# ctxnn/GenConViT

Hardware: AMD Instinct MI355X
Metric: frames/sec (224x224, ed+vae forward) (higher is better)
Workload: dtype f16

## Files before the change

### genconvit_amd/csrc/api.hip

```cpp
#include "../../include/genconvit_hip.h"

#include <dlfcn.h>

#include <cstdio>
#include <cstdlib>
#include <cstring>
#include <map>
#include <mutex>
#include <set>
#include <sstream>
#include <vector>

#include "fused_mlp.h"
#include "gemm.h"
#include "mlp_pair.h"
#include "xs_mlp.h"
#include "kernels.h"
#include "net.h"

namespace gcv {
static thread_local std::string g_err;
void set_error(const std::string& msg) { g_err = msg; }
const char* get_error() { return g_err.c_str(); }

// ... 144 lines not shown
  a.lnp_w = l->w; a.lnp_b = l->b; a.lnp_eps = l->eps; a.lnp_nseg = l->nseg;
  for (int i = 0; i < l->nseg && i < 4; ++i) {
    a.lnp_tok0[i] = l->tok0[i]; a.lnp_hw[i] = l->hw[i]; a.lnp_wd[i] = l->wd[i]; a.lnp_out0[i] = l->out0[i];
  }
}
template <typename T>
static int k_mlp_dispatch(int C, const void* x, const void* w1, const float* b1, const float* w2_f32, const float* b2,
                          const float* gamma, const void* resid, void* out, int M, hipStream_t s, int iters = 0,
                          float* ms = nullptr, const LnpSpec* lnp = nullptr) {
  struct DevBuf {
    void* p = nullptr;
    hipStream_t s;
    explicit DevBuf(hipStream_t st) : s(st) {}
    ~DevBuf() { if (p) { (void)hipStreamSynchronize(s); (void)hipFree(p); } }
  };
  struct Ev {
    hipEvent_t e = nullptr;
    ~Ev() { if (e) (void)hipEventDestroy(e); }
  };
  DevBuf w2c(s), w1f(s), hid(s);
  GCV_CHECK_HIP(hipMalloc(&w2c.p, (size_t)4 * C * C * 2));
  auto timed = [&](auto&& f, float* avg) -> int {
    if (iters <= 0) return f();
    Ev e0, e1;
    GCV_CHECK_HIP(hipEventCreate(&e0.e));
    GCV_CHECK_HIP(hipEventCreate(&e1.e));
    GCV_TRY(f());
    GCV_CHECK_HIP(hipEventRecord(e0.e, s));
    for (int i = 0; i < iters; ++i) GCV_TRY(f());
    GCV_CHECK_HIP(hipEventRecord(e1.e, s));
    GCV_CHECK_HIP(hipEventSynchronize(e1.e));
    float t = 0.0f;
    GCV_CHECK_HIP(hipEventElapsedTime(&t, e0.e, e1.e));
    if (avg) *avg = t / (float)iters;
    return 0;
  };
  if (ms) ms[0] = ms[1] = ms[2] = 0.0f;
  if (lnp) {
    GCV_REQUIRE(lnp->nseg >= 1 && lnp->nseg <= 4 && lnp->w && lnp->b && lnp->tok0 && lnp->hw && lnp->wd && lnp->out0,
                "fused MLP with LN-patchify epilogue: 1..4 segments and their tables");
    GCV_REQUIRE((C == 96 && fused_mlp_res_applies(C, M)) || xs_mlp_default(C),
                "the LN-patchify epilogue exists at C = 96 (M >= 65536 tokens) and C = 192");
    int64_t covered = 0;
    for (int i = 0; i < lnp->nseg; ++i) {
      const int end = i + 1 < lnp->nseg ? lnp->tok0[i + 1] : M;
      const int wd = lnp->wd[i], hw = lnp->hw[i];
      GCV_REQUIRE(wd > 0 && hw > 0 && hw % wd == 0 && wd % 2 == 0 && (hw / wd) % 2 == 0 && lnp->tok0[i] == covered &&
                      end > lnp->tok0[i] && (end - lnp->tok0[i]) % hw == 0 && lnp->out0[i] * 4 == lnp->tok0[i],
                  "LN-patchify segments: contiguous whole images with even height and width");
      covered = end;
    }
  }
  if (mlp_pair_supported(C)) {
    GCV_CHECK_HIP(hipMalloc(&w1f.p, (size_t)4 * C * C * 2));
    GCV_CHECK_HIP(hipMalloc(&hid.p, mlp_pair_hidden_bytes(M, C)));
    GCV_TRY((launch_pack_w1_frag<T, T>((const T*)w1, (T*)w1f.p, C, s)));
    GCV_TRY((launch_pack_w2_frag<T, float>(w2_f32, gamma, (T*)w2c.p, C, s)));
    MlpPairArgs a{x, w1f.p, b1, w2c.p, b2, gamma, resid, out, hid.p, M};
    if (iters > 0) {
      GCV_TRY(timed([&] { return launch_xs_pw1<T>(a, C, s); }, ms ? ms + 1 : nullptr));
      GCV_TRY(timed([&] { return launch_pw2f<T>(a, C, s); }, ms ? ms + 2 : nullptr));
    }
    return timed([&] { return launch_mlp_pair<T>(a, C, s); }, ms);
  }
  static const bool legacy = exp_env("GCV_MLP_LEGACY") != nullptr;
  if (xs_mlp_default(C) && !legacy) {
    GCV_CHECK_HIP(hipMalloc(&w1f.p, xs_mlp_packed_elems(C) * sizeof(T)));
    GCV_TRY((launch_pack_xs_mlp<T, float>((const T*)w1, w2_f32, (T*)w1f.p, C, s)));
    XsMlpArgs xa{x, w1f.p, b1, b2, gamma, resid, out, M};
    set_lnp(xa, lnp);
    return timed([&] { return launch_xs_mlp<T>(xa, C, s); }, ms);
  }
  MlpArgs a{x, w1, b1, w2c.p, b2, gamma, resid, out, M};
  set_lnp(a, lnp);
  GCV_TRY(launch_pack_w2_chunks<T>(w2_f32, (T*)w2c.p, C, s));
  return timed([&] { return launch_fused_mlp<T>(a, C, s); }, ms);
}

extern "C" {

const char* gcv_last_error(void) { return get_error(); }

struct DeviceGuard {
  int prev = -1;
  explicit DeviceGuard(int dev) {
    if (hipGetDevice(&prev) != hipSuccess) prev = -1;
    if (prev != dev) (void)hipSetDevice(dev); else prev = -1;
  }
  ~DeviceGuard() { if (prev >= 0) (void)hipSetDevice(prev); }
};

int gcv_create(gcv_handle** out, int device, int dtype, int max_batch) {
  GCV_REQUIRE(out != nullptr, "null handle pointer");
  *out = nullptr;
  GCV_REQUIRE(max_batch >= 1 && max_batch <= 512, "max_batch must be in [1,512]");
  int ndev = 0;
  GCV_CHECK_HIP(hipGetDeviceCount(&ndev));
  GCV_REQUIRE(device >= 0 && device < ndev, "no such HIP device");
  hipDeviceProp_t prop;
  GCV_CHECK_HIP(hipGetDeviceProperties(&prop, device));
  GCV_REQUIRE(std::string(prop.gcnArchName).rfind("gfx950", 0) == 0,
              std::string("kernels are built for gfx950 only, device is ") + prop.gcnArchName);
  NetBase* net = nullptr;
  switch (dtype) {
    case GCV_F32:  net = make_net_f32(); break;
    case GCV_BF16: net = make_net_bf16(); break;
    case GCV_F16:  net = make_net_f16(); break;
    default: set_error("dtype must be GCV_F32, GCV_BF16 or GCV_F16"); return -2;
  }
  net->device = device;
  net->dtype = dtype;
// ... 401 lines not shown
```

### genconvit_amd/csrc/gemm.h

```cpp
#pragma once
#include <type_traits>

#include "common.h"

namespace gcv {

enum { A_PLAIN = 0, A_IM2COL3_POOL = 1, A_IM2COL3_S2 = 2 };
enum { EPI_BIAS_ACT = 0, EPI_RESID = 1, EPI_POOL4 = 2, EPI_CONVT = 3, EPI_SPLITK = 4 };

struct GemmArgs {
  const void* A;
  const void* Wt;
  void* C;
  const float* bias;
  const float* gamma;
  const void* resid;
  float* partial;
  int M, N, K;
  int lda, ldc;
  int act;
  int splitk;
  int k_per_split;
  int H, W;
  int cin_log2;
  int cout_log2;
};

typedef float f32x4 __attribute__((ext_vector_type(4)));
typedef float f32x16 __attribute__((ext_vector_type(16)));
typedef _Float16 f16x8 __attribute__((ext_vector_type(8)));
typedef __bf16 bf16x8 __attribute__((ext_vector_type(8)));

template <typename T> struct Mfma;
template <> struct Mfma<float> {
  __device__ static __forceinline__ void run(const u32x4& a, const u32x4& b, f32x16& acc) {
    const f32x4 af = __builtin_bit_cast(f32x4, a), bf = __builtin_bit_cast(f32x4, b);
#pragma unroll
    for (int j = 0; j < 4; ++j) acc = __builtin_amdgcn_mfma_f32_32x32x2f32(af[j], bf[j], acc, 0, 0, 0);
  }
};
template <> struct Mfma<half_t> {
  __device__ static __forceinline__ void run(const u32x4& a, const u32x4& b, f32x16& acc) {
    acc = __builtin_amdgcn_mfma_f32_32x32x16_f16(__builtin_bit_cast(f16x8, a), __builtin_bit_cast(f16x8, b), acc, 0, 0, 0);
  }
};
template <> struct Mfma<bf16_t> {
  __device__ static __forceinline__ void run(const u32x4& a, const u32x4& b, f32x16& acc) {
    acc = __builtin_amdgcn_mfma_f32_32x32x16_bf16(__builtin_bit_cast(bf16x8, a), __builtin_bit_cast(bf16x8, b), acc, 0, 0, 0);
  }
};

__device__ __forceinline__ float erf_fast(float x) {
  const float a = fabsf(x);
  const float t = __builtin_amdgcn_rcpf(fmaf(0.3275911f, a, 1.0f));
  float p = fmaf(1.061405429f, t, -1.453152027f);
  p = fmaf(p, t, 1.421413741f);
  p = fmaf(p, t, -0.284496736f);
  p = fmaf(p, t, 0.254829592f);
  p *= t;
  const float e = __builtin_amdgcn_exp2f(a * a * -1.4426950408889634f);
  return copysignf(fmaf(-p, e, 1.0f), x);
// ... 518 lines not shown
```

### genconvit_amd/csrc/gemm_bf16.hip

```cpp
#include "gemm_impl.h"
namespace gcv { template int launch_gemm<bf16_t>(const GemmArgs&, int, int, hipStream_t); }
```

### genconvit_amd/csrc/gemm_f16.hip

```cpp
#include "gemm_impl.h"
namespace gcv { template int launch_gemm<half_t>(const GemmArgs&, int, int, hipStream_t); }

GCV_GLDS_STAMP_READER
```

### genconvit_amd/csrc/gemm_glds.h

```cpp
#pragma once
#include "gemm.h"

namespace gcv {

#ifndef GCV_GLDS_STAGES
#define GCV_GLDS_STAGES 2
#endif
constexpr int kGldsBM = 128, kGldsBN = 192;
template <int BKB> struct GldsRing { static constexpr int stages = BKB == 64 ? GCV_GLDS_STAGES : 2; };

template <typename T, int BKB = 64> struct GldsSmem {
  static constexpr int kStage = (kGldsBM + kGldsBN) * BKB;
  static constexpr int kMain = GldsRing<BKB>::stages * kStage;
  static constexpr int kEpiRow = kGldsBN / 2 + 4;
  static constexpr int kEpiBG = kGldsBM * kEpiRow * 4;
  static constexpr int kEpi = kEpiBG + 2 * kGldsBN * 4;
  static constexpr int bytes = kMain > kEpi ? kMain : kEpi;
};

template <typename T, int EPI, int ACT, int BKB = 64>
__global__ void __launch_bounds__(256, 2) gemm_glds_kernel(const GemmArgs g) {
  static_assert(sizeof(T) == 2, "LDS-DMA GEMM is built for 16-bit storage");
  static_assert(EPI == EPI_BIAS_ACT || EPI == EPI_RESID, "epilogues: bias+act, layer-scale residual");
  static_assert(BKB == 64 || BKB == 128, "LDS rows are 64 or 128 bytes");
  constexpr int BM = kGldsBM, BN = kGldsBN, S = GldsRing<BKB>::stages;
  constexpr int EPC = 8, CPR = BKB / 16, BK = CPR * EPC;
  constexpr int RPI = 64 / CPR;
  constexpr int STAGE = GldsSmem<T, BKB>::kStage;
  auto swz = [](int row) { return CPR == 4 ? ((row >> 2) & 3) : ((row >> 1) & 7); };
  constexpr int A_BYTES = BM * BKB;
  constexpr int NQ = STAGE / 1024;
  constexpr int QPW = NQ / 4;
  constexpr int MI = 2, NI = 3;

  extern __shared__ __attribute__((aligned(16))) unsigned char smem[];

  const int tid = threadIdx.x;
  const int lane = tid & 63;
  const int wave = __builtin_amdgcn_readfirstlane(tid >> 6);
  const int lr = lane & 31, lh = lane >> 5;
  const int wm0 = (wave >> 1) * 64, wn0 = (wave & 1) * 96;

  GLDS_STAMP(0);
  GLDS_STAMP_HWID();
  const int ntn = g.N / BN;
  const int ntm = (g.M + BM - 1) / BM;
  const int bid = xcd_remap(blockIdx.x, ntm * ntn);
  const int m0 = (bid / ntn) * BM;
  const int n0 = (bid % ntn) * BN;
  const int nkt = g.K / BK;

  const T* src[QPW];
#pragma unroll
  for (int i = 0; i < QPW; ++i) {
    const int q = wave + 4 * i;
    const int rl = q * RPI + lane / CPR;
    const int phys = lane % CPR;
    if (rl < BM) {
      const int c = phys ^ swz(rl);
      const int m = min(m0 + rl, g.M - 1);
      src[i] = (const T*)g.A + (int64_t)m * g.lda + c * EPC;
    } else {
      const int rb = rl - BM;
      const int c = phys ^ swz(rb);
      const int n = min(n0 + rb, g.N - 1);
      src[i] = (const T*)g.Wt + (int64_t)n * g.K + c * EPC;
    }
  }
  auto issue = [&](int kt) {
    unsigned char* base = smem + (kt % S) * STAGE;
#pragma unroll
    for (int i = 0; i < QPW; ++i) {
      const int q = wave + 4 * i;
      __builtin_amdgcn_global_load_lds((const __attribute__((address_space(1))) void*)(src[i] + (int64_t)kt * BK),
                                       (__attribute__((address_space(3))) void*)(base + q * 1024), 16, 0, 0);
    }
// ... 59 lines not shown
  for (int s = 0; s < S - 1; ++s)
    if (s < nkt) issue(s);
  const int n_steady = nkt - (S - 2) > 0 ? nkt - (S - 2) : 0;
  for (int kt = 0; kt < n_steady; ++kt) {
    asm volatile("s_waitcnt vmcnt(%0)\n\ts_barrier" ::"n"((S - 2) * QPW) : "memory");
    if (kt == 0) GLDS_STAMP(1);
    if (!(GCV_GLDS_ABLATE & 2) && kt + S - 1 < nkt) issue(kt + S - 1);
    if (!(GCV_GLDS_ABLATE & 1)) compute(kt);
  }
  for (int kt = n_steady; kt < nkt; ++kt) {
    asm volatile("s_waitcnt vmcnt(0)\n\ts_barrier" ::: "memory");
    if (!(GCV_GLDS_ABLATE & 1)) compute(kt);
  }
  asm volatile("s_waitcnt lgkmcnt(0)\n\ts_barrier" ::: "memory");
  GLDS_STAMP(2);

  constexpr int SROW = GldsSmem<T, BKB>::kEpiRow;
  uint32_t* sC = reinterpret_cast<uint32_t*>(smem);
  float* sBG = reinterpret_cast<float*>(smem + GldsSmem<T, BKB>::kEpiBG);
  T* Cp = (T*)g.C;
  if (EPI == EPI_RESID && !RESID_EARLY && !(GCV_GLDS_ABLATE & 4)) load_resid();
  if (tid < BN / 2) *(f32x4*)(sBG + 4 * tid) = pre;
  __syncthreads();
#pragma unroll
  for (int j = 0; j < NI; ++j) {
#pragma unroll
    for (int q = 0; q < 4; ++q) {
      const int nl = wn0 + j * 32 + 8 * q + 4 * lh;
      const f32x4 bv = *(const f32x4*)(sBG + nl);
      f32x4 gv = {1.f, 1.f, 1.f, 1.f};
      if (EPI == EPI_RESID) gv = *(const f32x4*)(sBG + BN + nl);
      float v[MI][4];
#pragma unroll
      for (int i = 0; i < MI; ++i)
#pragma unroll
        for (int e = 0; e < 4; ++e) v[i][e] = acc[i][j][4 * q + e];
      if (!(GCV_GLDS_ABLATE & 4)) bias_act4n<ACT, T, MI>(v, bv);
#pragma unroll
      for (int i = 0; i < MI; ++i) {
        const int ml = wm0 + i * 32 + lr;
        if (EPI == EPI_RESID && !(GCV_GLDS_ABLATE & 4)) {
          const t4 r = rres[i][j][q];
#pragma unroll
          for (int e = 0; e < 4; ++e) v[i][e] = fmaf(v[i][e], gv[e], to_f(r[e]));
        }
        t4 o = {from_f<T>(v[i][0]), from_f<T>(v[i][1]), from_f<T>(v[i][2]), from_f<T>(v[i][3])};
        *(t4*)(sC + ml * SROW + (nl >> 1)) = o;
      }
    }
  }
  GLDS_STAMP(3);
  __syncthreads();
  constexpr int PPR = BN / 8;
#pragma unroll 4
  for (int idx = tid; idx < BM * PPR; idx += 256) {
    const int rl = idx / PPR, pc = idx - rl * PPR;
    const int m = m0 + rl;
    if (m < g.M) *(u32x4*)(Cp + (int64_t)m * g.ldc + n0 + 8 * pc) = *(const u32x4*)(sC + rl * SROW + 4 * pc);
  }
  GLDS_STAMP(4);
#if GCV_GLDS_STAMPS
  asm volatile("s_waitcnt vmcnt(0)" ::: "memory");
  GLDS_STAMP(6);
#endif
}

template <typename T> int launch_gemm_glds(const GemmArgs& g, int epi, hipStream_t s);
template <typename T> bool gemm_glds_applicable(const GemmArgs& g, int a_mode, int epi);

}
```

### genconvit_amd/csrc/gemm_glds_impl.h

```cpp
#pragma once
#include <cstdlib>

#include "gemm_glds.h"

namespace gcv {

template <typename T, int EPI, int ACT, int BKB> static int launch_glds_bkb(const GemmArgs& g, hipStream_t s) {
  constexpr int SMEM = GldsSmem<T, BKB>::bytes;
  GCV_ENSURE_LDS((gemm_glds_kernel<T, EPI, ACT, BKB>), SMEM);
  const int ntm = cdiv(g.M, kGldsBM), ntn = g.N / kGldsBN;
  hipLaunchKernelGGL((gemm_glds_kernel<T, EPI, ACT, BKB>), dim3(ntm * ntn), dim3(256), SMEM, s, g);
  GCV_CHECK_HIP(hipGetLastError());
  return 0;
}

template <typename T, int EPI, int ACT> static int launch_glds_cfg(const GemmArgs& g, hipStream_t s) {
  static const bool line64 = exp_env("GCV_GLDS_ROW64") != nullptr;
  if (g.K % 64 == 0 && g.K >= 512 && !line64) return launch_glds_bkb<T, EPI, ACT, 128>(g, s);
  return launch_glds_bkb<T, EPI, ACT, 64>(g, s);
}

template <typename T> bool gemm_glds_applicable(const GemmArgs& g, int a_mode, int epi) {
  static const bool disabled = exp_env("GCV_NO_GLDS") != nullptr;
  if (disabled || sizeof(T) != 2 || a_mode != A_PLAIN) return false;
  if (!(epi == EPI_BIAS_ACT && (g.act == ACT_NONE || g.act == ACT_GELU)) && !(epi == EPI_RESID && g.act == ACT_NONE))
    return false;
  if (g.N % kGldsBN != 0 || g.K % 32 != 0 || g.M < 256 || g.lda % 8 != 0 || g.ldc % 8 != 0) return false;
  auto al = [](const void* p, unsigned a) { return (reinterpret_cast<uintptr_t>(p) % a) == 0; };
  if (!al(g.A, 16) || !al(g.Wt, 16) || !al(g.C, 16) || (g.bias && !al(g.bias, 16))) return false;
  if (epi == EPI_RESID && (!g.gamma || !g.resid || !al(g.gamma, 16) || !al(g.resid, 8))) return false;
  return true;
}

template <typename T> int launch_gemm_glds(const GemmArgs& g, int epi, hipStream_t s) {
  if (epi == EPI_RESID) return launch_glds_cfg<T, EPI_RESID, ACT_NONE>(g, s);
  if (g.act == ACT_GELU) return launch_glds_cfg<T, EPI_BIAS_ACT, ACT_GELU>(g, s);
  return launch_glds_cfg<T, EPI_BIAS_ACT, ACT_NONE>(g, s);
}

}
```

### genconvit_amd/csrc/mlp_pair.h

```cpp
#pragma once
#include <type_traits>

#include "gemm.h"

namespace gcv {

struct MlpPairArgs {
  const void* X;
  const void* W1f;
  const float* b1;
  const void* W2f;
  const float* b2;
  const float* gamma;
  const void* resid;
  void* out;
  void* hidden;
  int M;
};

template <typename T, typename S>
__global__ void __launch_bounds__(256) pack_w1_frag_kernel(const S* __restrict__ w1, T* __restrict__ out, int C) {
  const int64_t total = (int64_t)4 * C * C;
  const int64_t i = (int64_t)blockIdx.x * 256 + threadIdx.x;
  if (i >= total) return;
// ... 426 lines not shown
    constexpr int lo = kc - (D - 2) > 0 ? kc - (D - 2) : 0, hi = kc < NPR ? kc : NPR;
    constexpr int WAITR = (D - 2) * PPW + (hi > lo ? hi - lo : 0);
    GCV_XS_WAIT(WAITR);
    if constexpr (kc >= RD) take_res(std::integral_constant<int, kc - RD>{});
    if constexpr (kc < NPR) issue_res(kc);
    __builtin_amdgcn_sched_barrier(0);
    compute(std::true_type{});
  });
#pragma unroll 1
  for (int kc = NPR + RD; kc < NSTEADY; ++kc) {
    if (kc >= 32 && kc < 40) P2_STAMP(4 * (kc - 32));
    GCV_XS_WAIT(WAITN);
    if (kc >= 32 && kc < 40) { P2_STAMP(4 * (kc - 32) + 1); P2_STAMP(4 * (kc - 32) + 2); }
    compute(std::true_type{});
    if (kc >= 32 && kc < 40) P2_STAMP(4 * (kc - 32) + 3);
  }
#pragma unroll
  for (int kc = NSTEADY; kc < NKC; ++kc) {
    asm volatile("s_waitcnt vmcnt(0)\n\ts_barrier" ::: "memory");
    compute(std::false_type{});
  }

  P2_STAMP(41);
  T* Op = (T*)a.out;
#pragma unroll
  for (int i = 0; i < MI; ++i) {
    const int64_t mm = row_of(i);
#pragma unroll
    for (int j = 0; j < NI; ++j)
#pragma unroll
      for (int pr = 0; pr < 2; ++pr) {
        uint2 pk[2];
#pragma unroll
        for (int d = 0; d < 2; ++d) {
          t4 o4;
#pragma unroll
          for (int e = 0; e < 4; ++e) o4[e] = from_f<T>(acc[i][j][4 * (2 * pr + d) + e]);
          pk[d] = __builtin_bit_cast(uint2, o4);
        }
        const auto sx = __builtin_amdgcn_permlane32_swap(pk[0].x, pk[1].x, false, false);
        const auto sy = __builtin_amdgcn_permlane32_swap(pk[0].y, pk[1].y, false, false);
        const u32x4 w = {sx[0], sy[0], sx[1], sy[1]};
        if (mm < a.M) *(u32x4*)(Op + mm * C + ncol0 + 32 * j + 16 * pr + 8 * lh) = w;
      }
  }
  P2_STAMP(42);
}

template <typename T> int launch_xs_pw1(const MlpPairArgs& a, int C, hipStream_t s);
template <typename T> int launch_pw2f(const MlpPairArgs& a, int C, hipStream_t s);
template <typename T> int launch_mlp_pair(const MlpPairArgs& a, int C, hipStream_t s);
template <typename T, typename S> int launch_pack_w1_frag(const S* w1, T* out, int C, hipStream_t s);
template <typename T, typename S> int launch_pack_w2_frag(const S* w2, const float* gamma, T* out, int C, hipStream_t s);
static inline bool mlp_pair_supported(int C) { return C == 384; }
static inline size_t mlp_pair_hidden_bytes(int64_t M, int C) { return (size_t)((M + 31) / 32) * (size_t)(4 * C / 32) * 2048; }

}
```

### genconvit_amd/csrc/mlp_pair_impl.h

```cpp
#pragma once
#include "mlp_pair.h"

namespace gcv {

template <typename T, typename S> int launch_pack_w1_frag(const S* w1, T* out, int C, hipStream_t s) {
  GCV_REQUIRE(C % 32 == 0, "pack_w1_frag: C must be a multiple of 32");
  const int64_t total = (int64_t)4 * C * C;
  hipLaunchKernelGGL((pack_w1_frag_kernel<T, S>), dim3((unsigned)cdiv64(total, 256)), dim3(256), 0, s, w1, out, C);
  GCV_CHECK_HIP(hipGetLastError());
  return 0;
}
template <typename T, typename S> int launch_pack_w2_frag(const S* w2, const float* gamma, T* out, int C, hipStream_t s) {
  GCV_REQUIRE(C % 32 == 0 && gamma, "pack_w2_frag: C must be a multiple of 32, gamma is folded into the packed weight");
  const int64_t total = (int64_t)4 * C * C;
  hipLaunchKernelGGL((pack_w2_frag_kernel<T, S>), dim3((unsigned)cdiv64(total, 256)), dim3(256), 0, s, w2, gamma, out, C);
  GCV_CHECK_HIP(hipGetLastError());
  return 0;
}

static inline int xs_pw1_pick_split(int ntile, int nkc) {
  int best = 1;
  long best_cost = -1;
  for (int ns = 1; ns <= 24; ++ns) {
    if (nkc % ns || (nkc / ns) % 2) continue;
    const long rounds = ((long)ntile * ns + 255) / 256;
    const long cost = rounds * (nkc / ns + 3);
    if (best_cost < 0 || cost < best_cost) { best_cost = cost; best = ns; }
  }
  return best;
}

static inline int mlp_pair_check(const MlpPairArgs& a, int C) {
  GCV_REQUIRE(a.M > 0 && a.X && a.W1f && a.W2f && a.b1 && a.b2 && a.gamma && a.resid && a.out && a.hidden,
              "MLP pair: null argument");
  GCV_REQUIRE(mlp_pair_supported(C), "MLP pair is built for C = 384");
  auto al = [](const void* p) { return (reinterpret_cast<uintptr_t>(p) & 15u) == 0; };
  GCV_REQUIRE(al(a.X) && al(a.W1f) && al(a.W2f) && al(a.b1) && al(a.resid) && al(a.out) && al(a.hidden),
              "MLP pair: operands must be 16-byte aligned");
  GCV_REQUIRE((int64_t)cdiv(a.M, 32) * (4 * C / 32) * 2048 < ((int64_t)1 << 31),
              "MLP pair: hidden tensor exceeds 32-bit buffer offsets");
  return 0;
}

template <typename T, int C> static int launch_xs_pw1_c(const MlpPairArgs& a, hipStream_t s) {
  constexpr int NKC = 4 * C / 32;
  constexpr int NW = 8, D = 6;
  constexpr int SMEM = XsPw1Smem<C, NW, D>::bytes;
  GCV_ENSURE_LDS((xs_pw1_kernel<T, C, NW, D>), SMEM);
  const int ntile = cdiv(a.M, 32 * NW);
  const int ns = xs_pw1_pick_split(ntile, NKC);
  GCV_REQUIRE((NKC / ns) % 2 == 0, "xs_pw1: an even number of hidden chunks per workgroup (two per barrier)");
  hipLaunchKernelGGL((xs_pw1_kernel<T, C, NW, D>), dim3(ntile, ns), dim3(NW * 64), SMEM, s, a, NKC / ns);
  GCV_CHECK_HIP(hipGetLastError());
  return 0;
}

template <typename T, int C, int BN, int D, int TB> static int launch_pw2f_cfg(const MlpPairArgs& a, hipStream_t s) {
  constexpr int SMEM = Pw2fSmem<C, BN, D, TB>::bytes;
  GCV_ENSURE_LDS((pw2f_kernel<T, C, BN, D, TB>), SMEM);
  hipLaunchKernelGGL((pw2f_kernel<T, C, BN, D, TB>), dim3(cdiv(a.M, 32 * TB) * (C / BN)), dim3(512), SMEM, s, a);
  GCV_CHECK_HIP(hipGetLastError());
  return 0;
}

template <typename T, int C> static int launch_pw2f_c(const MlpPairArgs& a, hipStream_t s) {
  const int ntm = cdiv(a.M, 256);
  if (ntm >= 180) return launch_pw2f_cfg<T, C, C, 3, 8>(a, s);
  if (ntm * (C / 192) >= 128) return launch_pw2f_cfg<T, C, 192, 4, 8>(a, s);
  return launch_pw2f_cfg<T, C, 192, 5, 4>(a, s);
}

template <typename T> int launch_xs_pw1(const MlpPairArgs& a, int C, hipStream_t s) {
  GCV_TRY(mlp_pair_check(a, C));
  return launch_xs_pw1_c<T, 384>(a, s);
}
template <typename T> int launch_pw2f(const MlpPairArgs& a, int C, hipStream_t s) {
  GCV_TRY(mlp_pair_check(a, C));
  return launch_pw2f_c<T, 384>(a, s);
}
template <typename T> int launch_mlp_pair(const MlpPairArgs& a, int C, hipStream_t s) {
  GCV_TRY(launch_xs_pw1<T>(a, C, s));
  return launch_pw2f<T>(a, C, s);
}

}
```

### genconvit_amd/csrc/net_impl.h

```cpp
#pragma once
#include <algorithm>
#include <cmath>
#include <cstdlib>
#include <cstring>

#include "cam.h"
#include "fused_mlp.h"
#include "mlp_pair.h"
#include "xs_mlp.h"
#include "gemm.h"
#include "kernels.h"
#include "net.h"
#include "swin.h"

namespace gcv {

template <typename T> inline T host_cvt(float v);
template <> inline float host_cvt<float>(float v) { return v; }
template <> inline half_t host_cvt<half_t>(float v) { return (half_t)v; }
template <> inline bf16_t host_cvt<bf16_t>(float v) {
  uint32_t u;
  std::memcpy(&u, &v, 4);
  uint16_t h;
  if ((u & 0x7fffffffu) > 0x7f800000u) h = (uint16_t)((u >> 16) | 0x40);
// ... 334 lines not shown
    GCV_UP(dst, st, o);
    return 0;
  }

  int pack_convnext(const TensorMap& w, const std::string& p, WeightStore& st, CnxW<T>& o) {
    {
      std::vector<float> v, t(48 * 96);
      GCV_TRY(fetch(w, p + "stem.0.weight", 96 * 48, v));
      for (int co = 0; co < 96; ++co)
        for (int k = 0; k < 48; ++k) t[k * 96 + co] = v[co * 48 + k];
      GCV_UP(o.stem_w, st, t);
    }
    GCV_TRY(up_f32(w, p + "stem.0.bias", 96, st, o.stem_b));
    GCV_TRY(up_f32(w, p + "stem.1.weight", 96, st, o.stem_lnw));
    GCV_TRY(up_f32(w, p + "stem.1.bias", 96, st, o.stem_lnb));
    int bi = 0;
    for (int i = 0; i < 4; ++i) {
      const int C = kDims[i];
      if (i > 0) {
        const int Cp = kDims[i - 1];
        const std::string d = p + "stages." + std::to_string(i) + ".downsample.";
        GCV_TRY(up_f32(w, d + "0.weight", Cp, st, o.down[i - 1].ln_w));
        GCV_TRY(up_f32(w, d + "0.bias", Cp, st, o.down[i - 1].ln_b));
        GCV_TRY(up_conv_gemm(w, d + "1.weight", C, Cp, 2, 2, nullptr, st, o.down[i - 1].w));
        GCV_TRY(up_f32(w, d + "1.bias", C, st, o.down[i - 1].b));
      }
      for (int j = 0; j < kDepths[i]; ++j, ++bi) {
        const std::string b = p + "stages." + std::to_string(i) + ".blocks." + std::to_string(j) + ".";
        CnxBlockW<T>& k = o.blk[bi];
        {
          std::vector<float> v, t((size_t)49 * C);
          GCV_TRY(fetch(w, b + "conv_dw.weight", (int64_t)C * 49, v));
          for (int c = 0; c < C; ++c)
            for (int q = 0; q < 49; ++q) t[(size_t)q * C + c] = v[(size_t)c * 49 + q];
          GCV_UP(k.dw_w, st, t);
        }
        GCV_TRY(up_f32(w, b + "conv_dw.bias", C, st, k.dw_b));
        GCV_TRY(up_f32(w, b + "norm.weight", C, st, k.ln_w));
        GCV_TRY(up_f32(w, b + "norm.bias", C, st, k.ln_b));
        GCV_TRY(up_cast(w, b + "mlp.fc1.weight", (int64_t)4 * C * C, st, k.fc1_w));
        GCV_TRY(up_f32(w, b + "mlp.fc1.bias", 4 * C, st, k.fc1_b));
        GCV_TRY(up_cast(w, b + "mlp.fc2.weight", (int64_t)4 * C * C, st, k.fc2_w));
        k.fc2_wc = nullptr;
        k.fc1_wf = k.fc2_wf = nullptr;
        k.fc_wp = nullptr;
        if constexpr (sizeof(T) == 2) {
          if (xs_mlp_default(C) && use_xs_mlp) {
            k.fc_wp = (T*)st.raw(xs_mlp_packed_elems(C) * sizeof(T));
            if (!k.fc_wp) { set_error("hipMalloc failed for the packed fc1 | fc2 records"); return -5; }
            GCV_TRY((launch_pack_xs_mlp<T, T>(k.fc1_w, k.fc2_w, k.fc_wp, C, nullptr)));
            GCV_CHECK_HIP(hipDeviceSynchronize());
          }
          if (mlp_pair_supported(C) && use_mlp_pair) {
            k.fc1_wf = (T*)st.raw((size_t)4 * C * C * sizeof(T));
            k.fc2_wf = (T*)st.raw((size_t)4 * C * C * sizeof(T));
            if (!k.fc1_wf || !k.fc2_wf) { set_error("hipMalloc failed for the fragment-major fc1 / fc2"); return -5; }
            GCV_TRY((launch_pack_w1_frag<T, T>(k.fc1_w, k.fc1_wf, C, nullptr)));
            {
              std::vector<float> v, gv;
              GCV_TRY(fetch(w, b + "mlp.fc2.weight", (int64_t)4 * C * C, v));
              GCV_TRY(fetch(w, b + "gamma", C, gv));
              struct DevBuf {
                float* p = nullptr;
                ~DevBuf() { if (p) (void)hipFree(p); }
              } tmp, tg;
              GCV_CHECK_HIP(hipMalloc((void**)&tmp.p, v.size() * 4));
              GCV_CHECK_HIP(hipMalloc((void**)&tg.p, gv.size() * 4));
              GCV_CHECK_HIP(hipMemcpy(tmp.p, v.data(), v.size() * 4, hipMemcpyHostToDevice));
              GCV_CHECK_HIP(hipMemcpy(tg.p, gv.data(), gv.size() * 4, hipMemcpyHostToDevice));
              GCV_TRY((launch_pack_w2_frag<T, float>(tmp.p, tg.p, k.fc2_wf, C, nullptr)));
              GCV_CHECK_HIP(hipDeviceSynchronize());
            }
          }
          if ((C <= 192 && !k.fc_wp) || (C == 384 && use_fused_mlp384)) {
            std::vector<float> v;
            GCV_TRY(fetch(w, b + "mlp.fc2.weight", (int64_t)4 * C * C, v));
            struct DevBuf {
              float* p = nullptr;
              ~DevBuf() { if (p) (void)hipFree(p); }
            } tmp;
            GCV_CHECK_HIP(hipMalloc((void**)&tmp.p, v.size() * 4));
            GCV_CHECK_HIP(hipMemcpy(tmp.p, v.data(), v.size() * 4, hipMemcpyHostToDevice));
            k.fc2_wc = (T*)st.raw(v.size() * sizeof(T));
            if (!k.fc2_wc) { set_error("hipMalloc failed for packed fc2"); return -5; }
            GCV_TRY(launch_pack_w2_chunks<T>(tmp.p, k.fc2_wc, C, nullptr));
            GCV_CHECK_HIP(hipDeviceSynchronize());
          }
        }
        GCV_TRY(up_f32(w, b + "mlp.fc2.bias", C, st, k.fc2_b));
        GCV_TRY(up_f32(w, b + "gamma", C, st, k.gamma));
      }
    }
    GCV_TRY(up_f32(w, p + "head.norm.weight", 768, st, o.head_lnw));
    GCV_TRY(up_f32(w, p + "head.norm.bias", 768, st, o.head_lnb));
    GCV_TRY(up_cast(w, p + "head.fc.weight", 1000 * 768, st, o.head_fc_w));
    GCV_TRY(up_f32(w, p + "head.fc.bias", 1000, st, o.head_fc_b));
    return 0;
  }

  int pack_head(const TensorMap& w, WeightStore& st, HeadW<T>& h) {
    GCV_TRY(up_cast(w, "fc.weight", 500 * 2000, st, h.fc_w));
    GCV_TRY(up_f32(w, "fc.bias", 500, st, h.fc_b));
    GCV_TRY(up_f32(w, "fc2.weight", 2 * 500, st, h.fc2_w));
    GCV_TRY(up_f32(w, "fc2.bias", 2, st, h.fc2_b));
    return 0;
  }

  int load_ed(const TensorMap& w) override {
    GCV_CHECK_HIP(hipSetDevice(device));
    has_ed = false;
// ... 190 lines not shown
        for (int s = 0; s < nseg;) {
          int e = s + 1, nimg = segs[s].n;
          int64_t mm = m[s];
          while (e < nseg && h[e] == h[s] && wd[e] == wd[s]) { nimg += segs[e].n; mm += m[e]; ++e; }
          GCV_TRY(run("cnx.dwconv7_ln", 2.0 * 49 * mm * C, 2.0 * sizeof(T) * (double)mm * C + 49.0 * C * 4, [&] {
            return launch_dwconv7_ln<T>(X + moff[s] * C, k.dw_w, k.dw_b, k.ln_w, k.ln_b, Y + moff[s] * C, nimg, h[s],
                                        wd[s], C, 1e-6f, cur);
          }));
          s = e;
        }
        if constexpr (sizeof(T) == 2) {
          if (k.fc_wp) {
            XsMlpArgs xa{Y, k.fc_wp, k.fc1_b, k.fc2_b, k.gamma, X, X, (int)M};
            if (j == kDepths[i] - 1 && i < 3 && use_lnp_epilogue) {
              bool even = true;
              int64_t o0 = 0;
              for (int s = 0; s < nseg; ++s) {
                xa.lnp_tok0[s] = (int)moff[s]; xa.lnp_hw[s] = h[s] * wd[s]; xa.lnp_wd[s] = wd[s]; xa.lnp_out0[s] = (int)o0;
                o0 += (int64_t)segs[s].n * (h[s] / 2) * (wd[s] / 2);
                even = even && h[s] % 2 == 0 && wd[s] % 2 == 0;
              }
              if (even) {
                xa.out = Hd; xa.lnp_w = w.down[i].ln_w; xa.lnp_b = w.down[i].ln_b; xa.lnp_eps = 1e-6f; xa.lnp_nseg = nseg;
                lnp_fused = true;
              }
            }
            GCV_TRY(run("cnx.fused_mlp", 16.0 * M * C * (double)C, 3.0 * sizeof(T) * (double)M * C + 16.0 * C * C,
                        [&] { return launch_xs_mlp<T>(xa, C, cur); }));
            GCV_TRY(tap_block(j));
            continue;
          }
          if (k.fc2_wc && use_fused_mlp && (C < 384 || use_fused_mlp384)) {
            MlpArgs ma{Y, k.fc1_w, k.fc1_b, k.fc2_wc, k.fc2_b, k.gamma, X, X, (int)M};
            if (j == kDepths[i] - 1 && i < 3 && use_lnp_epilogue && fused_mlp_res_applies(C, M)) {
              ma.out = Hd;
              ma.lnp_w = w.down[i].ln_w; ma.lnp_b = w.down[i].ln_b; ma.lnp_eps = 1e-6f; ma.lnp_nseg = nseg;
              int64_t o0 = 0;
              bool even = true;
              for (int s = 0; s < nseg; ++s) {
                ma.lnp_tok0[s] = (int)moff[s]; ma.lnp_hw[s] = h[s] * wd[s]; ma.lnp_wd[s] = wd[s]; ma.lnp_out0[s] = (int)o0;
                o0 += (int64_t)segs[s].n * (h[s] / 2) * (wd[s] / 2);
                even = even && h[s] % 2 == 0 && wd[s] % 2 == 0;
              }
              if (even) lnp_fused = true;
              else { ma.out = X; ma.lnp_nseg = 0; }
            }
            GCV_TRY(run("cnx.fused_mlp", 16.0 * M * C * (double)C, 3.0 * sizeof(T) * (double)M * C + 16.0 * C * C,
                        [&] { return launch_fused_mlp<T>(ma, C, cur); }));
            GCV_TRY(tap_block(j));
            continue;
          }
        }
        if constexpr (sizeof(T) == 2) {
          if (k.fc1_wf && k.fc2_wf) {
            MlpPairArgs pa{Y, k.fc1_wf, k.fc1_b, k.fc2_wf, k.fc2_b, k.gamma, X, X, Hd, (int)M};
            GCV_TRY(run("cnx.pw1_gelu", 8.0 * M * C * (double)C, sizeof(T) * (5.0 * M * C + 4.0 * C * C),
                        [&] { return launch_xs_pw1<T>(pa, C, cur); }));
            GCV_TRY(run("cnx.pw2_scale_res", 8.0 * M * C * (double)C, sizeof(T) * (6.0 * M * C + 4.0 * C * C),
                        [&] { return launch_pw2f<T>(pa, C, cur); }));
            GCV_TRY(tap_block(j));
            continue;
          }
        }
        GemmArgs g1{};
        g1.A = Y; g1.lda = C; g1.Wt = k.fc1_w; g1.C = Hd; g1.ldc = 4 * C; g1.bias = k.fc1_b;
        g1.M = (int)M; g1.N = 4 * C; g1.K = C; g1.act = ACT_GELU; g1.splitk = 1;
        GCV_TRY(gemm("cnx.pw1_gelu", g1, A_PLAIN, EPI_BIAS_ACT));
        GemmArgs g2{};
        g2.A = Hd; g2.lda = 4 * C; g2.Wt = k.fc2_w; g2.C = X; g2.ldc = C; g2.bias = k.fc2_b; g2.gamma = k.gamma;
        g2.resid = X; g2.M = (int)M; g2.N = C; g2.K = 4 * C; g2.act = ACT_NONE; g2.splitk = 1;
        GCV_TRY(gemm("cnx.pw2_scale_res", g2, A_PLAIN, EPI_RESID));
        GCV_TRY(tap_block(j));
      }
    }
    bool one_fc = nseg > 1;
    for (int s = 1; s < nseg && one_fc; ++s)
      one_fc = segs[s].n == segs[0].n && segs[s].out == segs[0].out + 1000 * s && segs[s].out_ld == 1000 * nseg &&
               segs[0].out_ld == 1000 * nseg && segs[s].act == segs[0].act;
    int no = 0;
    for (int s = 0; s < nseg; ++s) {
      if (s == 0 || h[s] * wd[s] != h[s - 1] * wd[s - 1]) {
        int e = s, nimg = 0;
        int64_t mm = 0;
        while (e < nseg && h[e] * wd[e] == h[s] * wd[s]) { nimg += segs[e].n; mm += m[e]; ++e; }
        GCV_TRY(run("cnx.pool_ln", 2.0 * mm * 768, sizeof(T) * (double)mm * 768, [&] {
          if (one_fc)
            return launch_pool_ln<T>(X + moff[s] * 768, w.head_lnw, w.head_lnb, Pool, nimg, h[s] * wd[s], 768, 1e-6f, cur,
                                     segs[0].n, nseg, s);
          return launch_pool_ln<T>(X + moff[s] * 768, w.head_lnw, w.head_lnb, Pool + (int64_t)no * 768, nimg, h[s] * wd[s],
                                   768, 1e-6f, cur);
        }));
      }
      if (!one_fc) {
        GemmArgs g{};
        g.A = Pool + (int64_t)no * 768; g.lda = 768; g.Wt = w.head_fc_w; g.C = segs[s].out; g.ldc = segs[s].out_ld;
        g.bias = w.head_fc_b; g.M = segs[s].n; g.N = 1000; g.K = 768; g.act = segs[s].act; g.splitk = 1;
        GCV_TRY(gemm("cnx.head_fc", g, A_PLAIN, EPI_BIAS_ACT));
        if (segs[s].pre) {
          g.C = segs[s].pre; g.act = ACT_NONE;
          GCV_TRY(gemm("explain.head_fc_pre", g, A_PLAIN, EPI_BIAS_ACT));
        }
      }
      no += segs[s].n;
    }
    if (tp) GCV_TRY(tap_bb(*tp, nseg, "pool", 3, 0, Pool, one_fc ? nseg : 0));
    if (one_fc) {
      GemmArgs g{};
// ... 317 lines not shown
```

### profiles/microbench.py

```python
#!/usr/bin/env python3
import ctypes, math, os, sys
import torch
ROOT = os.path.dirname(os.path.dirname(os.path.abspath(__file__)))
sys.path.insert(0, ROOT)
from genconvit_amd import _lib

which = sys.argv[1]
iters = int(sys.argv[2]) if len(sys.argv) > 2 else 20
dt, code = torch.float16, _lib.GCV_F16
dev = torch.device("cuda", 0)
lib = _lib.load()
st = lambda: _lib.current_stream_ptr(dev)
R = lambda *s: (torch.rand(*s, device=dev) * 2 - 1)
nimg = int(os.environ.get("GCV_MB_NIMG", "256"))


def run(fn, flops, bytes_):
    for _ in range(3):
        fn()
    torch.cuda.synchronize()
    e0, e1 = torch.cuda.Event(enable_timing=True), torch.cuda.Event(enable_timing=True)
    e0.record()
    for _ in range(iters):
        fn()
    e1.record()
    torch.cuda.synchronize()
    ms = e0.elapsed_time(e1) / iters
    print(f"{which}: {ms*1e3:.1f} us/launch  {flops/ms/1e9:.1f} TFLOP/s  {bytes_/ms/1e6:.1f} GB/s (algorithmic)")


if which.startswith("dwconv"):
    C = int(which[6:])
    H = {96: 56, 192: 28, 384: 14, 768: 7}[C]
    x = R(nimg, H, H, C).to(dt)
    y = torch.empty_like(x)
    w, b, lw, lb = R(49, C), R(C), R(C) + 1.5, R(C)
    fn = lambda: _lib.check(lib.gcv_k_dwconv7_ln(code, x.data_ptr(), w.data_ptr(), b.data_ptr(), lw.data_ptr(),
                                                 lb.data_ptr(), y.data_ptr(), nimg, H, H, C, 1e-6, st()), "dw")
    n = nimg * H * H * C
    run(fn, 2.0 * 49 * n, 4.0 * n)
elif which.startswith("mlp"):
    C = int(which[3:])
    H = {96: 56, 192: 28, 384: 14}[C]
    M = nimg * H * H
    x = R(M, C).to(dt)
    res = R(M, C).to(dt)
    w1 = (R(4 * C, C) / math.sqrt(C)).to(dt)
    w2 = R(C, 4 * C) / math.sqrt(4 * C)
    b1, b2, g = R(4 * C), R(C), R(C)
    ms3 = (ctypes.c_float * 3)()
    _lib.check(lib.gcv_k_fused_mlp_timed(code, C, x.data_ptr(), w1.data_ptr(), b1.data_ptr(), w2.data_ptr(), b2.data_ptr(),
                                         g.data_ptr(), res.data_ptr(), res.data_ptr(), M, iters, ms3, st()), "mlp")
    ms = ms3[0]
    extra = f"  (pw1 {ms3[1]*1e3:.1f} us, pw2 {ms3[2]*1e3:.1f} us)" if ms3[1] > 0 else ""
    print(f"{which}: {ms*1e3:.1f} us/launch  {16.0*M*C*C/ms/1e9:.1f} TFLOP/s  {6.0*M*C/ms/1e6:.1f} GB/s (algorithmic){extra}")
else:
    kind, C = which.split("_")
    C = int(C)
    H = {96: 56, 192: 28, 384: 14, 768: 7}[C]
    M = nimg * H * H
    if kind == "pw1":
        N, K, epi, act = 4 * C, C, _lib.EPI_BIAS_ACT, _lib.ACT_GELU
    else:
        N, K, epi, act = C, 4 * C, _lib.EPI_RESID, _lib.ACT_NONE
    A = R(M, K).to(dt)
    W = (R(N, K) / math.sqrt(K)).to(dt)
    Cm = R(M, N).to(dt)
    bias, gamma = R(N), R(N)
    g = _lib.GemmArgs(A.data_ptr(), W.data_ptr(), Cm.data_ptr(), bias.data_ptr(), gamma.data_ptr(), Cm.data_ptr(), None,
                      M, N, K, K, N, act, 1, 0, 0, 0, 0, 0)
    fn = lambda: _lib.check(lib.gcv_k_gemm(code, _lib.A_PLAIN, epi, ctypes.byref(g), st()), "gemm")
    run(fn, 2.0 * M * N * K, 2.0 * (M * K + N * K + M * N * (2 if kind == "pw2" else 1)))
```

Measured before the change: 17110.

## Extend MLP pair path to C=768 with fragment-major GELU GEMM epilogue

Enables the paired MLP path for the C=768 ConvNeXt stage. The first pointwise GEMM now uses the LDS-DMA GEMM with a new epilogue that writes the hidden activation directly in the fragment-major layout the fused pw2 kernel expects. The aim is to cut the cost of the token-major hidden round-trip and use the specialised pw2 kernel at the last stage. The path is gated on a minimum token count, and the pw2 tile configuration is adjusted so the 384-specific config is not used at 768.

```diff
diff --git a/genconvit_amd/csrc/api.hip b/genconvit_amd/csrc/api.hip
--- a/genconvit_amd/csrc/api.hip
+++ b/genconvit_amd/csrc/api.hip
@@ -220,11 +220,13 @@
     }
   }
   if (mlp_pair_supported(C)) {
-    GCV_CHECK_HIP(hipMalloc(&w1f.p, (size_t)4 * C * C * 2));
     GCV_CHECK_HIP(hipMalloc(&hid.p, mlp_pair_hidden_bytes(M, C)));
-    GCV_TRY((launch_pack_w1_frag<T, T>((const T*)w1, (T*)w1f.p, C, s)));
+    if (C == 384) {
+      GCV_CHECK_HIP(hipMalloc(&w1f.p, (size_t)4 * C * C * 2));
+      GCV_TRY((launch_pack_w1_frag<T, T>((const T*)w1, (T*)w1f.p, C, s)));
+    }
     GCV_TRY((launch_pack_w2_frag<T, float>(w2_f32, gamma, (T*)w2c.p, C, s)));
-    MlpPairArgs a{x, w1f.p, b1, w2c.p, b2, gamma, resid, out, hid.p, M};
+    MlpPairArgs a{x, C == 384 ? w1f.p : w1, b1, w2c.p, b2, gamma, resid, out, hid.p, M};
     if (iters > 0) {
       GCV_TRY(timed([&] { return launch_xs_pw1<T>(a, C, s); }, ms ? ms + 1 : nullptr));
       GCV_TRY(timed([&] { return launch_pw2f<T>(a, C, s); }, ms ? ms + 2 : nullptr));
diff --git a/genconvit_amd/csrc/gemm.h b/genconvit_amd/csrc/gemm.h
--- a/genconvit_amd/csrc/gemm.h
+++ b/genconvit_amd/csrc/gemm.h
@@ -6,7 +6,8 @@
 namespace gcv {
 
 enum { A_PLAIN = 0, A_IM2COL3_POOL = 1, A_IM2COL3_S2 = 2 };
-enum { EPI_BIAS_ACT = 0, EPI_RESID = 1, EPI_POOL4 = 2, EPI_CONVT = 3, EPI_SPLITK = 4 };
+enum { EPI_BIAS_ACT = 0, EPI_RESID = 1, EPI_POOL4 = 2, EPI_CONVT = 3, EPI_SPLITK = 4,
+       EPI_HFRAG = 5 };
 
 struct GemmArgs {
   const void* A;
diff --git a/genconvit_amd/csrc/gemm_bf16.hip b/genconvit_amd/csrc/gemm_bf16.hip
--- a/genconvit_amd/csrc/gemm_bf16.hip
+++ b/genconvit_amd/csrc/gemm_bf16.hip
@@ -1,2 +1,5 @@
 #include "gemm_impl.h"
-namespace gcv { template int launch_gemm<bf16_t>(const GemmArgs&, int, int, hipStream_t); }
+namespace gcv {
+template int launch_gemm<bf16_t>(const GemmArgs&, int, int, hipStream_t);
+template int launch_gemm_glds_hfrag<bf16_t>(const GemmArgs&, hipStream_t);
+}
diff --git a/genconvit_amd/csrc/gemm_f16.hip b/genconvit_amd/csrc/gemm_f16.hip
--- a/genconvit_amd/csrc/gemm_f16.hip
+++ b/genconvit_amd/csrc/gemm_f16.hip
@@ -1,4 +1,7 @@
 #include "gemm_impl.h"
-namespace gcv { template int launch_gemm<half_t>(const GemmArgs&, int, int, hipStream_t); }
+namespace gcv {
+template int launch_gemm<half_t>(const GemmArgs&, int, int, hipStream_t);
+template int launch_gemm_glds_hfrag<half_t>(const GemmArgs&, hipStream_t);
+}
 
 GCV_GLDS_STAMP_READER
diff --git a/genconvit_amd/csrc/gemm_glds.h b/genconvit_amd/csrc/gemm_glds.h
--- a/genconvit_amd/csrc/gemm_glds.h
+++ b/genconvit_amd/csrc/gemm_glds.h
@@ -21,7 +21,8 @@
 template <typename T, int EPI, int ACT, int BKB = 64>
 __global__ void __launch_bounds__(256, 2) gemm_glds_kernel(const GemmArgs g) {
   static_assert(sizeof(T) == 2, "LDS-DMA GEMM is built for 16-bit storage");
-  static_assert(EPI == EPI_BIAS_ACT || EPI == EPI_RESID, "epilogues: bias+act, layer-scale residual");
+  static_assert(EPI == EPI_BIAS_ACT || EPI == EPI_RESID || EPI == EPI_HFRAG,
+                "epilogues: bias+act (token-major or fragment-major), layer-scale residual");
   static_assert(BKB == 64 || BKB == 128, "LDS rows are 64 or 128 bytes");
   constexpr int BM = kGldsBM, BN = kGldsBN, S = GldsRing<BKB>::stages;
   constexpr int EPC = 8, CPR = BKB / 16, BK = CPR * EPC;
@@ -187,6 +188,21 @@
   GLDS_STAMP(3);
   __syncthreads();
   constexpr int PPR = BN / 8;
+  if constexpr (EPI == EPI_HFRAG) {
+    const int nkc = g.N / 32, ntb = (g.M + 31) >> 5;
+    const int tb0 = m0 >> 5, kc0 = n0 >> 5;
+    constexpr int PPT = BN / 32 * 128;
+#pragma unroll 4
+    for (int idx = tid; idx < BM * PPR; idx += 256) {
+      const int tbl = idx / PPT, rem = idx - tbl * PPT;
+      const int kcl = rem >> 7, kq = (rem >> 5) & 3, tok = rem & 31;
+      if (tb0 + tbl < ntb)
+        *(u32x4*)((unsigned char*)g.C + ((int64_t)(tb0 + tbl) * nkc + kc0 + kcl) * 2048 + (rem & 127) * 16) =
+            *(const u32x4*)(sC + (tbl * 32 + tok) * SROW + (kcl * 32 + kq * 8) / 2);
+    }
+    GLDS_STAMP(4);
+    return;
+  }
 #pragma unroll 4
   for (int idx = tid; idx < BM * PPR; idx += 256) {
     const int rl = idx / PPR, pc = idx - rl * PPR;
@@ -201,6 +217,7 @@
 }
 
 template <typename T> int launch_gemm_glds(const GemmArgs& g, int epi, hipStream_t s);
+template <typename T> int launch_gemm_glds_hfrag(const GemmArgs& g, hipStream_t s);
 template <typename T> bool gemm_glds_applicable(const GemmArgs& g, int a_mode, int epi);
 
 }
diff --git a/genconvit_amd/csrc/gemm_glds_impl.h b/genconvit_amd/csrc/gemm_glds_impl.h
--- a/genconvit_amd/csrc/gemm_glds_impl.h
+++ b/genconvit_amd/csrc/gemm_glds_impl.h
@@ -38,4 +38,12 @@
   return launch_glds_cfg<T, EPI_BIAS_ACT, ACT_NONE>(g, s);
 }
 
+template <typename T> int launch_gemm_glds_hfrag(const GemmArgs& g, hipStream_t s) {
+  GCV_REQUIRE(g.act == ACT_GELU && g.N % kGldsBN == 0 && g.K % 64 == 0 && g.K >= 512 && g.M > 0 && g.lda % 8 == 0,
+              "fragment-major GELU GEMM: N % 192 == 0, K % 64 == 0, K >= 512");
+  auto al = [](const void* p) { return (reinterpret_cast<uintptr_t>(p) & 15u) == 0; };
+  GCV_REQUIRE(al(g.A) && al(g.Wt) && al(g.C) && g.bias && al(g.bias), "fragment-major GELU GEMM: 16-byte aligned operands");
+  return launch_glds_bkb<T, EPI_HFRAG, ACT_GELU, 128>(g, s);
 }
+
+}
diff --git a/genconvit_amd/csrc/mlp_pair.h b/genconvit_amd/csrc/mlp_pair.h
--- a/genconvit_amd/csrc/mlp_pair.h
+++ b/genconvit_amd/csrc/mlp_pair.h
@@ -502,7 +502,8 @@
 template <typename T> int launch_mlp_pair(const MlpPairArgs& a, int C, hipStream_t s);
 template <typename T, typename S> int launch_pack_w1_frag(const S* w1, T* out, int C, hipStream_t s);
 template <typename T, typename S> int launch_pack_w2_frag(const S* w2, const float* gamma, T* out, int C, hipStream_t s);
-static inline bool mlp_pair_supported(int C) { return C == 384; }
+static inline bool mlp_pair_supported(int C) { return C == 384 || C == 768; }
+constexpr int kMlpPair768MinM = 4096;
 static inline size_t mlp_pair_hidden_bytes(int64_t M, int C) { return (size_t)((M + 31) / 32) * (size_t)(4 * C / 32) * 2048; }
 
 }
diff --git a/genconvit_amd/csrc/mlp_pair_impl.h b/genconvit_amd/csrc/mlp_pair_impl.h
--- a/genconvit_amd/csrc/mlp_pair_impl.h
+++ b/genconvit_amd/csrc/mlp_pair_impl.h
@@ -1,4 +1,5 @@
 #pragma once
+#include "gemm_glds.h"
 #include "mlp_pair.h"
 
 namespace gcv {
@@ -33,7 +34,7 @@
 static inline int mlp_pair_check(const MlpPairArgs& a, int C) {
   GCV_REQUIRE(a.M > 0 && a.X && a.W1f && a.W2f && a.b1 && a.b2 && a.gamma && a.resid && a.out && a.hidden,
               "MLP pair: null argument");
-  GCV_REQUIRE(mlp_pair_supported(C), "MLP pair is built for C = 384");
+  GCV_REQUIRE(mlp_pair_supported(C), "MLP pair is built for C = 384 and C = 768");
   auto al = [](const void* p) { return (reinterpret_cast<uintptr_t>(p) & 15u) == 0; };
   GCV_REQUIRE(al(a.X) && al(a.W1f) && al(a.W2f) && al(a.b1) && al(a.resid) && al(a.out) && al(a.hidden),
               "MLP pair: operands must be 16-byte aligned");
@@ -65,17 +66,25 @@
 
 template <typename T, int C> static int launch_pw2f_c(const MlpPairArgs& a, hipStream_t s) {
   const int ntm = cdiv(a.M, 256);
-  if (ntm >= 180) return launch_pw2f_cfg<T, C, C, 3, 8>(a, s);
+  if constexpr (C == 384)
+    if (ntm >= 180) return launch_pw2f_cfg<T, C, C, 3, 8>(a, s);
   if (ntm * (C / 192) >= 128) return launch_pw2f_cfg<T, C, 192, 4, 8>(a, s);
   return launch_pw2f_cfg<T, C, 192, 5, 4>(a, s);
 }
 
 template <typename T> int launch_xs_pw1(const MlpPairArgs& a, int C, hipStream_t s) {
   GCV_TRY(mlp_pair_check(a, C));
+  if (C == 768) {
+    GemmArgs g{};
+    g.A = a.X; g.lda = C; g.Wt = a.W1f; g.C = a.hidden; g.ldc = 4 * C; g.bias = a.b1;
+    g.M = a.M; g.N = 4 * C; g.K = C; g.act = ACT_GELU; g.splitk = 1;
+    return launch_gemm_glds_hfrag<T>(g, s);
+  }
   return launch_xs_pw1_c<T, 384>(a, s);
 }
 template <typename T> int launch_pw2f(const MlpPairArgs& a, int C, hipStream_t s) {
   GCV_TRY(mlp_pair_check(a, C));
+  if (C == 768) return launch_pw2f_c<T, 768>(a, s);
   return launch_pw2f_c<T, 384>(a, s);
 }
 template <typename T> int launch_mlp_pair(const MlpPairArgs& a, int C, hipStream_t s) {
diff --git a/genconvit_amd/csrc/net_impl.h b/genconvit_amd/csrc/net_impl.h
--- a/genconvit_amd/csrc/net_impl.h
+++ b/genconvit_amd/csrc/net_impl.h
@@ -410,10 +410,10 @@
             GCV_CHECK_HIP(hipDeviceSynchronize());
           }
           if (mlp_pair_supported(C) && use_mlp_pair) {
-            k.fc1_wf = (T*)st.raw((size_t)4 * C * C * sizeof(T));
+            k.fc1_wf = C == 384 ? (T*)st.raw((size_t)4 * C * C * sizeof(T)) : k.fc1_w;
             k.fc2_wf = (T*)st.raw((size_t)4 * C * C * sizeof(T));
             if (!k.fc1_wf || !k.fc2_wf) { set_error("hipMalloc failed for the fragment-major fc1 / fc2"); return -5; }
-            GCV_TRY((launch_pack_w1_frag<T, T>(k.fc1_w, k.fc1_wf, C, nullptr)));
+            if (C == 384) GCV_TRY((launch_pack_w1_frag<T, T>(k.fc1_w, k.fc1_wf, C, nullptr)));
             {
               std::vector<float> v, gv;
               GCV_TRY(fetch(w, b + "mlp.fc2.weight", (int64_t)4 * C * C, v));
@@ -710,7 +710,7 @@
           }
         }
         if constexpr (sizeof(T) == 2) {
-          if (k.fc1_wf && k.fc2_wf) {
+          if (k.fc1_wf && k.fc2_wf && (C == 384 || M >= kMlpPair768MinM)) {
             MlpPairArgs pa{Y, k.fc1_wf, k.fc1_b, k.fc2_wf, k.fc2_b, k.gamma, X, X, Hd, (int)M};
             GCV_TRY(run("cnx.pw1_gelu", 8.0 * M * C * (double)C, sizeof(T) * (5.0 * M * C + 4.0 * C * C),
                         [&] { return launch_xs_pw1<T>(pa, C, cur); }));
diff --git a/profiles/microbench.py b/profiles/microbench.py
--- a/profiles/microbench.py
+++ b/profiles/microbench.py
@@ -41,7 +41,7 @@
     run(fn, 2.0 * 49 * n, 4.0 * n)
 elif which.startswith("mlp"):
     C = int(which[3:])
-    H = {96: 56, 192: 28, 384: 14}[C]
+    H = {96: 56, 192: 28, 384: 14, 768: 7}[C]
     M = nimg * H * H
     x = R(M, C).to(dt)
     res = R(M, C).to(dt)
```

Result: no change. 17180 (median of 6 runs) (+0.4%).
